# feihoo87/waveforms

Hardware: AMD Instinct MI355X
Metric: Msamples/s (all channels) (higher is better)
Workload: dtype f64; 1 GPU; sampler256: 256 ch/GPU x 1e+07 pts, 100 gaussian+DRAG pulses/ch, seeds 1000+c (SURVEY 8(d) C4/C5 channel spec), grid mode; channels_per_gpu=256, channels_total=256, points_per_channel=10000000, output=device (HBM) buffer, parallelism=channel-block-per-rank x1, no data-path collective

## Files before the change

### include/wfk.h

```cpp
#ifndef WFK_H
#define WFK_H

#include <stddef.h>
#include <stdint.h>

#ifdef __cplusplus
extern "C" {
#endif

#define WFK_ABI_VERSION 2

#define WFK_OK 0
#define WFK_EINVAL (-1)
#define WFK_EUNSUP (-2)
#define WFK_EHIP   (-3)
#define WFK_ENOMEM (-4)
#define WFK_ETIMEOUT (-5)

enum {
  WFK_LINEAR = 1, WFK_GAUSSIAN = 2, WFK_ERF = 3, WFK_COS = 4, WFK_SINC = 5,
  WFK_EXP = 6, WFK_INTERP = 7, WFK_LINEARCHIRP = 8, WFK_EXPONENTIALCHIRP = 9,
  WFK_HYPERBOLICCHIRP = 10, WFK_COSH = 11, WFK_SINH = 12, WFK_DRAG = 13,
  WFK_MOLLIFIER = 14, WFK_D_GAUSSIAN = 15, WFK_DRAG_SIN = 16, WFK_DRAG_SINX = 17,
  WFK_SAMPLED = 1000
// ... 55 lines not shown

int wfk_plan_create_grid(const wfk_program* prog, const wfk_grid* grid,
                         wfk_plan** out);
int wfk_plan_create_tlist(const wfk_program* prog, const double* t_host,
                          int64_t n, wfk_plan** out);
int wfk_grid_detect(const double* t_host, int64_t n, wfk_grid* grid);
int wfk_grid_detect_runs(const double* t_host, int64_t n, int64_t min_len, int32_t max_runs,
                         int64_t* starts, wfk_grid* grids);
int wfk_plan_destroy(wfk_plan* plan);
int wfk_plan_get_info(const wfk_plan* plan, wfk_plan_info* info);
int wfk_plan_member_index(const wfk_plan* plan, int32_t member, int64_t* idx,
                          int32_t cap);
int wfk_plan_channel_is_complex(const wfk_plan* plan, int32_t channel);
const char* wfk_plan_kernel_name(const wfk_plan* plan, int out_kind);
int64_t wfk_plan_table_bytes(const wfk_plan* plan);
int wfk_plan_launch(wfk_plan* plan, void* out_dev, int64_t ch_stride,
                    int out_kind, uint32_t flags, void* hip_stream);
int wfk_plan_run_host(wfk_plan* plan, void* out_host, int64_t ch_stride,
                      int out_kind);

int wfk_fir_plan_create(const double* ker_host, int32_t K, int64_t n,
                        int32_t batch, int kind ,
                        wfk_fir_plan** out);
int wfk_fir_plan_create_rows(const double* kers_host, int32_t K, int64_t n,
                             int32_t batch, int kind ,
                             wfk_fir_plan** out);
int wfk_fir_apply(wfk_fir_plan* plan, const void* in_dev, int64_t in_stride,
                  void* out_dev, int64_t out_stride, void* hip_stream);
int wfk_fir_plan_destroy(wfk_fir_plan* plan);

// ... 119 lines not shown
```

### waveforms_amd/_engine.py

```python
from __future__ import annotations

import ctypes as C
import importlib.util
import os

import numpy as np

from ._flatten import Program, wfk_grid, wfk_program

_HERE = os.path.dirname(os.path.abspath(__file__))
LIB_PATH = os.environ.get('WFK_LIB') or os.path.join(_HERE, 'csrc', 'libwfk_hip.so')

OUT_F64, OUT_F32, OUT_C128, OUT_C64 = 0, 1, 2, 3
ACCUMULATE = 1
_KIND_OF = {np.dtype(np.float64): OUT_F64, np.dtype(np.float32): OUT_F32,
            np.dtype(np.complex128): OUT_C128, np.dtype(np.complex64): OUT_C64}
_DTYPE_OF = {v: k for k, v in _KIND_OF.items()}

E_UNSUP = -2
E_TIMEOUT = -5


class wfk_plan_info(C.Structure):
    _fields_ = [('n_channels', C.c_int32), ('n', C.c_int64), ('tile', C.c_int32),
# ... 22 lines not shown
        l = C.CDLL(LIB_PATH)
        l.wfk_last_error.restype = C.c_char_p
        P, I64, I32, VP = C.POINTER, C.c_int64, C.c_int32, C.c_void_p
        l.wfk_plan_create_grid.argtypes = [P(wfk_program), P(wfk_grid), P(VP)]
        l.wfk_plan_create_tlist.argtypes = [P(wfk_program), VP, I64, P(VP)]
        l.wfk_grid_detect.argtypes = [VP, I64, P(wfk_grid)]
        l.wfk_grid_detect_runs.argtypes = [VP, I64, I64, I32, VP, P(wfk_grid)]
        l.wfk_plan_destroy.argtypes = [VP]
        l.wfk_plan_get_info.argtypes = [VP, P(wfk_plan_info)]
        l.wfk_plan_member_index.argtypes = [VP, I32, VP, I32]
        l.wfk_plan_channel_is_complex.argtypes = [VP, I32]
        l.wfk_plan_kernel_name.argtypes = [VP, C.c_int]
        l.wfk_plan_kernel_name.restype = C.c_char_p
        l.wfk_plan_table_bytes.argtypes = [VP]
        l.wfk_plan_table_bytes.restype = C.c_int64
        l.wfk_plan_launch.argtypes = [VP, VP, I64, C.c_int, C.c_uint32, VP]
        l.wfk_plan_run_host.argtypes = [VP, VP, I64, C.c_int]
        l.wfk_fir_plan_create.argtypes = [VP, I32, I64, I32, C.c_int, P(VP)]
        l.wfk_fir_plan_create_rows.argtypes = [VP, I32, I64, I32, C.c_int, P(VP)]
        l.wfk_chain_plan_create_rows.argtypes = [P(wfk_program), P(wfk_grid), VP, I32, C.c_int, P(VP)]
        l.wfk_fir_apply.argtypes = [VP, VP, I64, VP, I64, VP]
        l.wfk_fir_plan_destroy.argtypes = [VP]
        l.wfk_chain_plan_create.argtypes = [P(wfk_program), P(wfk_grid), VP, I32, C.c_int, P(VP)]
        l.wfk_chain_is_fused.argtypes = [VP]
        l.wfk_chain_unfused_reason.argtypes = [VP]
        l.wfk_chain_unfused_reason.restype = C.c_char_p
        l.wfk_chain_kernel_name.argtypes = [VP]
        l.wfk_chain_kernel_name.restype = C.c_char_p
        l.wfk_chain_table_bytes.argtypes = [VP]
        l.wfk_chain_table_bytes.restype = I64
# ... 146 lines not shown
        self.n = int(info.n)
        self.n_channels = int(info.n_channels)

    def member_index(self, member: int) -> np.ndarray:
        nb = len(self.prog.member_bounds(member))
        idx = np.empty(nb, dtype=np.int64)
        check(lib().wfk_plan_member_index(self._h, member, idx.ctypes.data, nb))
        return idx

    def kernel_name(self, dtype=np.float64) -> str:
        return lib().wfk_plan_kernel_name(self._h, _KIND_OF[np.dtype(dtype)]).decode()

    def table_bytes(self) -> int:
        return int(lib().wfk_plan_table_bytes(self._h))

    def launch(self, out_ptr: int, ch_stride: int, kind: int, accumulate=False,
               stream: int = 0):
        check(lib().wfk_plan_launch(self._h, out_ptr, ch_stride, kind,
                                    ACCUMULATE if accumulate else 0, stream))

    def run_host(self, dtype=np.float64) -> np.ndarray:
        dtype = np.dtype(dtype)
        out = pinned_empty((self.n_channels, self.n), dtype)
        if out.size:
            check(lib().wfk_plan_run_host(self._h, out.ctypes.data, self.n,
                                          _KIND_OF[dtype]))
        return out

    def run_host_into(self, out: np.ndarray):
        if out.size != self.n_channels * self.n or not out.flags.c_contiguous or not out.flags.writeable:
# ... 407 lines not shown
```

### waveforms_amd/csrc/wfk_api.cpp

```cpp
#include <hip/hip_runtime.h>

#include <algorithm>
#include <cstring>
#include <map>
#include <mutex>
#include <thread>
#include <new>
#include <string>
#include <vector>

#include "wfk.h"
#include "wfk_host.h"
#include "wfk_internal.h"

static thread_local std::string g_err;

#define HIP_TRY(expr)                                                                 \
  do {                                                                                \
    hipError_t e_ = (expr);                                                           \
    if (e_ != hipSuccess)                                                             \
      return wfk_fail(WFK_EHIP, std::string(#expr) + ": " + hipGetErrorString(e_));   \
  } while (0)

namespace {
// ... 76 lines not shown
  }
};

struct wfk_plan {
  HostPlan h;
  bool on_device = false;
  void* d_tables = nullptr;
  size_t tables_cap = 0;
  DevChannel* d_channels = nullptr;
  DevPiece* d_pieces = nullptr;
  double* d_params = nullptr;
  double* d_pool = nullptr;
  int32_t* d_chunk_first = nullptr;
  int32_t* d_lean_chunk_first = nullptr;
  int32_t* d_f32_chunk_first = nullptr;
  double* d_tlist = nullptr;
  ShortUnit* d_units = nullptr;
  uint32_t* d_slots = nullptr;
  void* d_scratch = nullptr;
  size_t scratch_bytes = 0;
  size_t scratch_cap = 0;
  int dev = 0;
  bool async_launch = false;
};

static int plan_upload(wfk_plan* p, const double* tlist) {
  if (!wfk_have_device()) {
    p->on_device = false;
    return WFK_OK;
  }
  const HostPlan& h = p->h;
  DevTables t;
  const size_t o_ch = t.add(h.channels);
  const size_t o_pc = t.add(h.pieces.data(), h.shortp && !h.mixed ? 0 : h.pieces.size() * sizeof(DevPiece));
  const size_t o_pa = t.add(h.params), o_po = t.add(h.pool), o_cf = t.add(h.chunk_first);
  const size_t o_lf = t.add(h.lean_chunk_first), o_ff = t.add(h.f32_chunk_first);
  const size_t o_un = t.add(h.s_units), o_sl = t.add(h.s_slots);
  const size_t b_tl = tlist ? (size_t)h.n * sizeof(double) : 0;
  const size_t o_tl = t.reserve(b_tl), total = t.total();
  HIP_TRY(dev_cache().get(total, &p->d_tables, &p->tables_cap, &p->dev));
  char* base = static_cast<char*>(p->d_tables);
  p->d_channels = t.at<DevChannel>(base, o_ch);
  p->d_pieces = t.at<DevPiece>(base, o_pc);
  p->d_params = t.at<double>(base, o_pa);
  p->d_pool = t.at<double>(base, o_po);
  p->d_chunk_first = t.at<int32_t>(base, o_cf);
  p->d_lean_chunk_first = t.at<int32_t>(base, o_lf);
  p->d_f32_chunk_first = t.at<int32_t>(base, o_ff);
  p->d_units = t.at<ShortUnit>(base, o_un);
  p->d_slots = t.at<uint32_t>(base, o_sl);
  p->d_tlist = tlist ? t.at<double>(base, o_tl) : nullptr;
  const std::vector<char>& stage = t.image();
  if (o_tl) HIP_TRY(hipMemcpy(base, stage.data(), o_tl, hipMemcpyHostToDevice));
  if (b_tl) HIP_TRY(hipMemcpy(base + o_tl, tlist, b_tl, hipMemcpyHostToDevice));
  p->on_device = true;
  return WFK_OK;
}

extern "C" {

void wfk_internal_set_error(const char* msg) { g_err = msg ? msg : ""; }

int wfk_abi_version(void) { return WFK_ABI_VERSION; }

const char* wfk_last_error(void) { return g_err.c_str(); }
// ... 32 lines not shown
    if (grid && prog && prog->n_channels >= 32 && prog->n_pieces >= 8192) {
      int nt = (int)std::min<unsigned>(16u, std::max(1u, std::thread::hardware_concurrency()));
      if (const char* e = std::getenv("WFK_COMPILE_THREADS")) nt = std::atoi(e);
      nt = std::min(nt, prog->n_channels / 8);
      if (nt > 1) rc = wfk_compile_blocks(prog, grid, nt, p->h, err);
    }
    if (rc == WFK_RETRY_STD) rc = wfk_compile(prog, grid, tlist, n, p->h, err);
  } catch (...) {
    delete p;
    throw;
  }
  if (rc) {
    delete p;
    return wfk_fail(rc, err);
  }
  std::vector<double> grid_t;
  const char* nopw = std::getenv("WFK_NO_POINTWISE_GRID");
  if (grid && p->h.short_gave_up && grid->n > 0 && grid->n <= ((int64_t)1 << 24) && !(nopw && nopw[0] == '1')) {
    try {
      grid_t.resize((size_t)grid->n);
      wfk_internal_grid_times(grid, grid_t.data());
      HostPlan h2;
      std::string err2;
      TlistNsGuard ns_guard(WFK_NS_TLIST_SMALL);
      const int rc2 = wfk_compile(prog, nullptr, grid_t.data(), grid->n, h2, err2);
      if (rc2 == WFK_OK) {
        h2.grid_as_tlist = true;
        h2.t0 = p->h.t0; h2.step = p->h.step; h2.last = p->h.last;
        h2.has_last = p->h.has_last; h2.i0 = p->h.i0;
        p->h = std::move(h2);
// ... 36 lines not shown
}

int wfk_plan_create_tlist(const wfk_program* prog, const double* t_host, int64_t n,
                          wfk_plan** out) {
  if (!t_host && n > 0) return wfk_fail(WFK_EINVAL, "null t_host");
  static const double dummy = 0.0;
  return plan_create(prog, nullptr, t_host ? t_host : &dummy, n, out);
}

int wfk_plan_destroy(wfk_plan* p) {
  if (!p) return WFK_OK;
  if (p->d_tables || p->d_scratch) {
    DeviceGuard guard(p->dev);
    if (p->async_launch) (void)hipDeviceSynchronize();
    dev_cache().put(p->d_tables, p->tables_cap, p->dev);
    dev_cache().put(p->d_scratch, p->scratch_cap, p->dev);
  }
  delete p;
  return WFK_OK;
}

int wfk_plan_get_info(const wfk_plan* p, wfk_plan_info* info) {
  if (!p || !info) return wfk_fail(WFK_EINVAL, "null argument");
  info->n_channels = p->h.n_channels;
  info->n = p->h.n;
  info->tile = p->h.tile;
  info->n_tiles = p->h.shortp ? (int64_t)p->h.s_units.size() : p->h.chunks_per_ch * p->h.n_channels;
  info->n_pieces = (int32_t)p->h.pieces.size();
  info->param_doubles = (int64_t)p->h.params.size();
  info->n_fast = p->h.n_fast;
// ... 15 lines not shown
  if (!p || channel < 0 || channel >= p->h.n_channels) return wfk_fail(WFK_EINVAL, "bad channel");
  return p->h.channel_complex[channel];
}

void wfk_internal_plan_tables(const wfk_plan* p, const HostPlan** h, const double** d_params) {
  *h = p ? &p->h : nullptr;
  *d_params = p && p->on_device ? p->d_params : nullptr;
}

int64_t wfk_plan_table_bytes(const wfk_plan* p) {
  if (!p) return wfk_fail(WFK_EINVAL, "null plan");
  const HostPlan& h = p->h;
  size_t b = h.channels.size() * sizeof(DevChannel) + h.params.size() * sizeof(double) + h.pool.size() * sizeof(double);
  if (h.shortp) b += h.s_units.size() * sizeof(ShortUnit) + h.s_slots.size() * sizeof(uint32_t);
  if (!h.shortp || h.mixed) b += h.pieces.size() * sizeof(DevPiece) + (h.chunk_first.size() + h.lean_chunk_first.size()) * sizeof(int32_t);
  return (int64_t)b;
}

const char* wfk_plan_kernel_name(const wfk_plan* p, int out_kind) {
  if (!p || out_kind < 0 || out_kind > 3) return "";
  static thread_local std::string name;
  const char* T = (out_kind == WFK_OUT_F32 || out_kind == WFK_OUT_C64) ? "float" : "double";
  const char* cplx = (out_kind == WFK_OUT_C128 || out_kind == WFK_OUT_C64) ? "true" : "false";
  const HostPlan& h = p->h;
  const bool f32 = out_kind == WFK_OUT_F32 || out_kind == WFK_OUT_C64;
  auto general = [&](bool tl, bool g, bool d, int ns) {
    const std::string tail = std::string(cplx) + "," + (tl ? "true" : "false") + "," + (g ? "true" : "false") + "," +
                             (d ? "true" : "false") + "," + std::to_string(ns) + ">";
    return f32 && (tl || g || d) ? "wfk_sample_wide<" + tail : std::string("wfk_sample<") + T + "," + tail;
  };
  if (h.shortp) {
// ... 5 lines not shown
  }
  const std::string lean_name = std::string("wfk_sample_lean<") + T + "," + cplx + "," + std::to_string(h.ns) +
      (h.n_corr > 0 && out_kind != WFK_OUT_F32 && out_kind != WFK_OUT_C64
           ? std::string(",true,") + std::to_string(h.lean_fam >= 1 ? 1 : 0) + ">"
           : std::string(",false,") + std::to_string(h.lean_fam) + ">");
  if (!h.tlist && h.lean) {
    name = lean_name;
  } else {
    const bool tl_full = h.tlist && (h.n_direct > 0 || h.n_generic > 0);
    const bool direct = tl_full || (!h.tlist && h.n_direct > 0), generic = direct || (!h.tlist && h.n_generic > 0);
    name = general(h.tlist, generic, direct, h.ns);
    if (h.mixed && h.tlist) name = general(true, false, false, h.ns) + " + " + name;
    else if (h.mixed) name = lean_name + " + " + name;
  }
  return name.c_str();
}

static int plan_launch_part(wfk_plan* p, void* out_dev, int64_t ch_stride, int out_kind, uint32_t flags,
                            void* hip_stream, int part, int nparts, int64_t* s_lo, int64_t* s_hi) {
  if (!p || (!out_dev && p->h.n > 0)) return wfk_fail(WFK_EINVAL, "null plan or output");
  if (!p->on_device)
    return wfk_fail(WFK_EHIP, "plan has no device tables (no HIP device was visible at plan creation)");
  if (ch_stride < p->h.n) return wfk_fail(WFK_EINVAL, "ch_stride smaller than samples per channel");
  if (s_lo) { *s_lo = 0; *s_hi = p->h.n; }
  if (p->h.n == 0 || p->h.n_channels == 0) return WFK_OK;
  if (nparts > 1 && (p->h.n_channels != 1 || p->h.mixed)) return wfk_fail(WFK_EINVAL, "partial launch of a multi-channel or mixed plan");
  auto sub = [&](int64_t total, int64_t& base, int64_t& count) {
    base = total * part / nparts;
    count = total * (part + 1) / nparts - base;
  };
// ... 72 lines not shown
    a.mixed = 1;
  } else if (p->h.mixed && p->h.tlist) {
    KArgs l = a;
    l.mixed = 1;
    rc = wfk_launch_sampler(l, p->h.n_channels, out_kind, true, p->h.ns, false, false, false, hip_stream, err);
    if (rc) return wfk_fail(rc, err);
    a.mixed = 1;
  } else if (p->h.mixed) {
    KArgs l = a;
    l.mixed = 1;
    l.chunk_first = p->d_lean_chunk_first;
    l.chunks_per_ch = p->h.lean_chunks_per_ch;
    l.n_chunks = p->h.lean_chunks_per_ch * p->h.n_channels;
    l.tiles_per_chunk = p->h.lean_tiles_per_chunk;
    if (f32_lean) use_f32_chunks(l);
    rc = wfk_launch_sampler(l, p->h.n_channels, out_kind, false, p->h.ns, true, false, false, hip_stream, err);
    if (rc) return wfk_fail(rc, err);
    a.mixed = 1;
  }
  if (nparts > 1) {
    const int64_t all = a.n_chunks;
    sub(all, a.chunk_base, a.n_chunks);
    const int64_t tile = (int64_t)(p->h.lean ? 64 : WFK_WG) * p->h.ns, span = tile * a.tiles_per_chunk;
    if (s_lo) {
      *s_lo = std::min<int64_t>(p->h.n, a.chunk_base * span);
      *s_hi = std::min<int64_t>(p->h.n, (a.chunk_base + a.n_chunks) * span);
    }
    if (a.n_chunks == 0) return WFK_OK;
  }
  rc = wfk_launch_sampler(a, p->h.n_channels, out_kind, p->h.tlist, p->h.ns, p->h.lean,
                          p->h.n_generic > 0 || (p->h.tlist && p->h.n_direct > 0),
                          p->h.n_direct > 0 || (p->h.tlist && p->h.n_generic > 0),
                          hip_stream, err);
// ... 252 lines not shown
```

### waveforms_amd/csrc/wfk_compile.cpp

```cpp
#include <algorithm>
#include <chrono>
#include <cmath>
#include <cstdio>
#include <cstdlib>
#include <cstring>
#include <atomic>
#include <map>
#include <string>
#include <thread>
#include <vector>

#include "wfk.h"
#include "wfk_internal.h"

namespace {

struct TimeAxis {
  const wfk_grid* g;
  const double* t;
  int64_t n;
  double at(int64_t i) const {
    if (t) return t[i];
    if (g->has_last && i == g->n - 1) return g->last;
    volatile double m = (double)(i + g->i0) * g->step;
// ... 1996 lines not shown
  H.foreign_frac = frac_sum / (double)P->n_channels;
  H.pool_real = !H.pool.empty();
  if (H.pool.empty()) H.pool.assign(1, 0.0);
  if (H.shortp) {
    const int64_t nu = (int64_t)H.s_units.size();
    H.s_units_per_chunk = (int32_t)std::min<int64_t>(6, std::max<int64_t>(1, nu / 8192));
    if (const char* e = std::getenv("WFK_SH_UPC")) {
      const int v = std::atoi(e);
      if (v >= 1 && v <= 64) H.s_units_per_chunk = v;
    }
    if (H.s_slots.empty()) H.s_slots.push_back(0);
  }
  return WFK_OK;
}

namespace {

struct GridProbe {
  const double* t;
  int64_t n;
  double t0;
  double at(int64_t i, double step) const { return (double)i * step + t0; }
  int64_t first_mismatch(double step, int64_t a, int64_t b, int* sign) const {
    for (int64_t c = a; c < b; c += 1024) {
      const int64_t e = std::min(b, c + 1024);
      int bad = 0;
      const double dc = (double)c;
      const double* tc = t + c;
      const int len = (int)(e - c);
      for (int k = 0; k < len; ++k) bad |= ((dc + (double)k) * step + t0) != tc[k];
// ... 220 lines not shown
```

### waveforms_amd/csrc/wfk_internal.h

```cpp
#pragma once
#include <stdint.h>

#define WFK_WG 256
#define WFK_NS_GRID 16
#define WFK_NS_TLIST 8
#define WFK_NS_TLIST_SMALL 1
#define WFK_TLIST_SMALL_N (1 << 20)
#define WFK_LDS_DOUBLES 2048
#define WFK_FREC 10
#define WFK_BLK_HDR 2
#define WFK_TERM_HDR 4
#define WFK_OP_TERM 1
#define WFK_OP_FCE 2

#define WFK_FCE_REC 22
#define WFK_FCE_W 1
#define WFK_FCE_SREF 2
#define WFK_FCE_SLIN 3
#define WFK_FCE_DEG 4
#define WFK_FCE_PACK(deg, carrier, imag, env, f32ok) ((deg) | ((carrier) << 2) | ((imag) << 3) | ((env) << 4) | ((f32ok) << 6))
#define WFK_FCE_WORD(rec) (reinterpret_cast<const int*>(rec)[2 * WFK_FCE_DEG])
#define WFK_FCE_TABOFF(fl) (((fl) >> 8) & 0x7FF)
#define WFK_FCE_STOFF(fl) ((((fl) >> 19) & 63) * 128)
#define WFK_FCE_HAS_CS (1 << 25)
// ... 31 lines not shown
#endif
#ifndef WFK_LEAN_PAR
#define WFK_LEAN_PAR 896
#endif
#define WFK_CHAIN_PAR 2048
#ifndef WFK_LEAN_RESEED
#define WFK_LEAN_RESEED 8
#endif
#define WFK_LEAN_RESEED_F32 32
#ifndef WFK_LEAN_RESEED_CS
#define WFK_LEAN_RESEED_CS 64
#endif
#define WFK_LEAN_TPC 5
#define WFK_LEAN_TPC_F32 20

#define WFK_PF_HAS_TERMS 1
#define WFK_PF_LEAN 2

#define WFK_SH_R 16
#define WFK_SH_LCAP 1008
#define WFK_SH_SUB 4096
#define WFK_SH_FILL 1008
#define WFK_SH_ERFTAB 512
#define WFK_SH_OP1 12
#define WFK_SH_OP3 16
#define WFK_SH_LAST 64
#define WFK_PF_SHORT 4
#define WFK_SH_SLOT(drec16, o, len) \
  ((uint32_t)(drec16) | ((uint32_t)(o) << 16) | ((uint32_t)((len) - 1) << 26) | 0x80000000u)
#define WFK_SH_DREC_MAX 0xffff
// ... 57 lines not shown
  int64_t n;
  int64_t chunks_per_ch;
  int64_t n_chunks;
  int64_t chunk_base;
  int32_t tiles_per_chunk;
  int32_t accumulate;
  double t0, step, last;
  int32_t has_last, pad;
  int32_t lean_par, lean_ops;
  int32_t corr;
  int32_t reseed;
  int32_t lean_fam;
  int32_t wavepriv;
  int32_t mixed;
  int64_t i0;
};

#ifdef __cplusplus
#include <string>
#include <vector>
struct wfk_program;
struct wfk_grid;
struct wfk_plan;
struct wfk_fir_plan;

struct HostPlan {
  bool tlist = false;
  int32_t n_channels = 0;
  int64_t n = 0;
  double t0 = 0, step = 0, last = 0;
// ... 6 lines not shown
  std::vector<double> params, pool;
  std::vector<int32_t> chunk_first;
  std::vector<std::vector<int64_t>> member_idx;
  std::vector<uint8_t> channel_complex;
  int32_t n_fast = 0, n_direct = 0, n_fused = 0, n_generic = 0;
  int32_t n_corr = 0;
  bool lean = false;
  int32_t lean_fam = 0;
  bool mixed = false;
  int32_t lean_tile = 0, lean_tiles_per_chunk = 1;
  int64_t lean_chunks_per_ch = 0;
  std::vector<int32_t> lean_chunk_first;
  int32_t f32_tiles_per_chunk = 0;
  int64_t f32_chunks_per_ch = 0;
  std::vector<int32_t> f32_chunk_first;
  int32_t lean_par = 0, lean_ops = 0;
  bool shortp = false;
  int32_t max_block_len = 0;
  double foreign_frac = 0.0;
  double mean_piece_len = 0.0;
  bool short_gave_up = false;
  bool grid_as_tlist = false;
  bool short_has_fmul = false;
  int32_t short_fam = 0;
  bool short_corr = false;
  bool short_needs_corr = false;
  bool pool_real = false;
  std::vector<ShortUnit> s_units;
  std::vector<uint32_t> s_slots;
  int32_t s_lds_samples = 0, s_units_per_chunk = 1;
};

int wfk_compile(const wfk_program* prog, const wfk_grid* grid, const double* tlist,
                int64_t n, HostPlan& out, std::string& err);

int wfk_compile_geom(const wfk_program* prog, const wfk_grid* grid, int lane_stride, int ns,
                     HostPlan& out, std::string& err);
#define WFK_RETRY_STD 1
int wfk_compile_blocks(const wfk_program* prog, const wfk_grid* grid, int nthreads, HostPlan& out, std::string& err);

struct ShortWin {
  int64_t rec0;
  int64_t e0;
  int32_t cnt, pad;
  int32_t ccnt, pad2;
};
#define WFK_PLAN_FOREIGN_ONLY 0x80000000u
#define WFK_CW_ENTRY(drec, o, len) ((uint32_t)(drec) | ((uint32_t)(o) << 16) | ((uint32_t)((len) - 1) << 28))
int wfk_chain_windows(const HostPlan& H, int64_t n, int64_t hop, int64_t lead, int64_t half, int64_t npairs,
                      std::vector<ShortWin>& wins, std::vector<uint32_t>& entries, std::string& err);

void wfk_internal_keep_mixed_short(bool on);
void wfk_internal_tlist_ns(int ns);
void wfk_internal_grid_times(const wfk_grid* g, double* out);
void wfk_internal_no_short_fmul(bool on);

int wfk_launch_sampler(const KArgs& a, int32_t n_channels, int out_kind, bool tlist, int ns,
                       bool lean, bool generic, bool direct, void* stream, std::string& err);
int wfk_launch_short(const SArgs& a, int out_kind, void* stream, std::string& err);

extern "C" {
void wfk_internal_set_error(const char* msg);
void wfk_internal_plan_tables(const wfk_plan* p, const HostPlan** h, const double** d_params);
int wfk_internal_plan_launch_foreign(wfk_plan* p, void* out_dev, int64_t ch_stride, int out_kind, void* hip_stream);
void wfk_internal_fir_tables(const wfk_fir_plan* p, const void** kspec, const void** tw, int* fused, int* nseg,
                             int* K, int* lead);
int64_t wfk_internal_fir_krow(const wfk_fir_plan* p);
int wfk_internal_fir_fused_launch(int kind, const void* in, int64_t in_stride, void* out, int64_t out_stride,
                                  const void* hspec, const void* tw, int64_t n, int M, int K, int lead, int64_t nblk,
                                  int32_t batch, int accumulate, void* stream, int64_t hspec_row_stride);
int wfk_internal_fir_fused_len(void);
}
#endif
// ... 1 lines not shown
```

### waveforms_amd/csrc/wfk_kernels.hip

```cpp
#include <hip/hip_runtime.h>

#include <string>
#include <type_traits>
#include <utility>

#include "wfk.h"
#include "wfk_internal.h"

namespace {

__device__ __forceinline__ int uni(int v) { return __builtin_amdgcn_readfirstlane(v); }
__device__ __forceinline__ int64_t uni64(int64_t v) {
  const uint32_t lo = __builtin_amdgcn_readfirstlane((uint32_t)v);
  const uint32_t hi = __builtin_amdgcn_readfirstlane((uint32_t)((uint64_t)v >> 32));
  return (int64_t)(((uint64_t)hi << 32) | lo);
}
#define WFK_CONST __attribute__((address_space(4)))
template <typename V>
__device__ __forceinline__ V cload(const void* base, int byte_off) {
  return *reinterpret_cast<const WFK_CONST V*>(reinterpret_cast<uintptr_t>(base) + byte_off);
}
__device__ __forceinline__ DevPiece load_piece(const DevPiece* p) {
  DevPiece P;
  P.start = cload<int64_t>(p, offsetof(DevPiece, start));
// ... 1179 lines not shown
  const bool full = P.start <= w0 && P.stop >= w0 + 64 * NS;
  const bool clip = C.do_clip && (P.flags & WFK_PF_HAS_TERMS);
  if (full && !clip && !a.accumulate)
    store_tile_impl<T, CPLX, NS, true, NT, E>(a, C, P, tr, tc, w0, lane, acc, acci);
  else
    store_tile_impl<T, CPLX, NS, false, NT, E>(a, C, P, tr, tc, w0, lane, acc, acci);
}

__device__ __forceinline__ int64_t xcd_chunk(const KArgs& a) {
  const int64_t b = blockIdx.x;
  const int64_t per = (a.n_chunks + 7) >> 3;
  const int64_t c = (b & 7) * per + (b >> 3);
  return c < a.n_chunks ? a.chunk_base + c : -1;
}

template <typename T, bool CPLX, int NS, bool CORR, int FAM>
#ifndef WFK_LEAN_WAVES
#define WFK_LEAN_WAVES 3
#endif
#ifndef WFK_LEAN_WAVES_F32
#define WFK_LEAN_WAVES_F32 4
#endif
__global__ void __launch_bounds__(64, (sizeof(T) == 4 ? WFK_LEAN_WAVES_F32 : WFK_LEAN_WAVES) - (CPLX ? 1 : 0) -
                                          (CORR && sizeof(T) == 8 && !CPLX ? 1 : 0))
wfk_sample_lean(const KArgs a) {
  extern __shared__ __attribute__((aligned(16))) double s_dyn[];
  double* const s_par = s_dyn;
  double* const s_st = s_dyn + a.lean_par;
  constexpr int WT = 64 * NS;
  using OutR = typename OutOps<T>::Real;
  using OutC = typename OutOps<T>::Cplx;

  const int lane = threadIdx.x;
  const int64_t chunk = xcd_chunk(a);
  if (chunk < 0) return;
  const int ch = uni((int)(chunk / a.chunks_per_ch));
  const int64_t cc = uni64(chunk - (int64_t)ch * a.chunks_per_ch);
  const DevChannel C = a.channels[ch];
  int p = uni(a.chunk_first[chunk]);
  DevPiece cur = load_piece(a.pieces + p);
  int64_t staged = -1;
  int state_piece = -1;
  int64_t state_w0 = -1;
  int since_seed = 0;
  int cs_age = 0;

  OutR* const outr = uniptr(reinterpret_cast<OutR*>(a.out) + (int64_t)ch * a.ch_stride);
  OutC* const outc = uniptr(reinterpret_cast<OutC*>(a.out) + (int64_t)ch * a.ch_stride);

  for (int tt = 0; tt < a.tiles_per_chunk; ++tt) {
    const int64_t w0 = uni64((cc * a.tiles_per_chunk + tt) * WT);
    if (w0 >= a.n) break;
    const int64_t w1 = w0 + WT < a.n ? w0 + WT : a.n;
    const int64_t j0 = w0 + lane;
    while (p < C.piece_end - 1 && cur.stop <= w0) {
      p = uni(p + 1);
      cur = load_piece(a.pieces + p);
    }

    for (int q = p;;) {
      const DevPiece P = cur;
      if (P.start >= w1) break;
      T acc[NS], acci[CPLX ? NS : 1];
      WFK_EACH(NS, k) acc[k] = (T)0; WFK_END
      WFK_EACH(CPLX ? NS : 1, k) acci[k] = (T)0; WFK_END
      const bool mine = !a.mixed || P.n_blk == 0 || (P.flags & WFK_PF_LEAN);
      if (P.n_blk != 0 && mine) {
        if (P.par_off != staged) {
          __syncthreads();
          for (int i = lane; i < P.first_len; i += 64) s_par[i] = a.params[P.par_off + i];
          __syncthreads();
          staged = P.par_off;
        }
        const int nops = uni((int)s_par[1]);
        double x = grid_time(a, j0);
        if (C.tshift != 0.0) x = x - C.tshift;
        const bool valid = state_piece == q && state_w0 == w0;
        const bool carried = valid && since_seed < a.reseed;
        if (!carried) {
          bool seed_cs = true;
          if constexpr (!CORR) {
            seed_cs = !valid || cs_age >= WFK_LEAN_RESEED_CS;
          }
          if (seed_cs) cs_age = 0;
          for (int op = 0; op < nops; ++op) {
            const double* srec = s_par + WFK_BLK_HDR + op * WFK_FCE_REC;
            const int sfl = uni(WFK_FCE_WORD(srec));
            if constexpr (!CORR) {
              if (!seed_cs && (sfl & (WFK_FCE_HAS_CS | WFK_FCE_HAS_GR | WFK_FCE_CHIRP)) == WFK_FCE_HAS_CS) continue;
            }
            if constexpr (FAM >= 2) {
              if (sfl & WFK_FCE_CHIRP) {
                const ChirpSeeds cd = chirp_make_seeds(srec, x, sfl);
                double* ct = s_st + WFK_FCE_STOFF(sfl) + lane;
                ct[0] = cd.c; ct[64] = cd.s; ct[128] = cd.wc; ct[192] = cd.ws;
                if (sfl & WFK_FCE_HAS_GR) { ct[256] = cd.g; ct[320] = cd.r; }
                continue;
              }
            }
            if constexpr (FAM >= 3) {
              if ((sfl & 0x32) == 0x32) continue;
            }
            const FceSeeds sd = fce_make_seeds<CORR>(srec, x, sfl);
// ... 311 lines not shown
    if (TLIST && !generic && !direct) { hipLaunchKernelGGL((wfk_sample_wide<CPLX, TLIST, false, false, NS>), g, b, 0, s, a); return hipGetLastError() == hipSuccess ? 0 : -1; }
    if (TLIST || direct) { hipLaunchKernelGGL((wfk_sample_wide<CPLX, TLIST, true, true, NS>), g, b, 0, s, a); return hipGetLastError() == hipSuccess ? 0 : -1; }
    if (generic) { hipLaunchKernelGGL((wfk_sample_wide<CPLX, false, true, false, NS>), g, b, 0, s, a); return hipGetLastError() == hipSuccess ? 0 : -1; }
  }
  if (TLIST && !generic && !direct)
    hipLaunchKernelGGL((wfk_sample<T, CPLX, TLIST, false, false, NS>), g, b, 0, s, a);
  else if (TLIST || direct)
    hipLaunchKernelGGL((wfk_sample<T, CPLX, TLIST, true, true, NS>), g, b, 0, s, a);
  else if (generic)
    hipLaunchKernelGGL((wfk_sample<T, CPLX, false, true, false, NS>), g, b, 0, s, a);
  else
    hipLaunchKernelGGL((wfk_sample<T, CPLX, false, false, false, NS>), g, b, 0, s, a);
  return hipGetLastError() == hipSuccess ? 0 : -1;
}

}

int wfk_launch_sampler(const KArgs& a, int32_t n_channels, int out_kind, bool tlist, int ns, bool lean,
                       bool generic, bool direct, void* stream, std::string& err) {
  if (a.chunk_base < 0 || a.chunk_base + a.n_chunks > (int64_t)n_channels * a.chunks_per_ch) { err = "chunk range outside the plan"; return WFK_EINVAL; }
  const int64_t blocks = ((a.n_chunks + 7) >> 3) << 3;
  if (blocks == 0) return WFK_OK;
  if (blocks > 0x7fffffffLL) { err = "grid too large"; return WFK_EINVAL; }
  hipStream_t s = (hipStream_t)stream;
  int rc;
  if (!tlist) {
    switch (out_kind) {
      case WFK_OUT_F64: rc = launch<double, false, false, WFK_NS_GRID>(a, blocks, s, lean, generic, direct); break;
      case WFK_OUT_F32: rc = launch<float, false, false, WFK_NS_GRID>(a, blocks, s, lean, generic, direct); break;
      case WFK_OUT_C128: rc = launch<double, true, false, WFK_NS_GRID>(a, blocks, s, lean, generic, direct); break;
// ... 24 lines not shown
```

Before: 805,900 Msamples/s.

## Precompute per-chunk oscillator and envelope seeds in a cached device table

Adds a pre-pass kernel that, on first launch, computes libm-based cos/sin/gaussian seeds at each lean chunk's first sample and stores them in a persistent device table. The main kernel's first reseed per chunk then reads the table and derives per-lane values with angle-doubling rotations and truncated Taylor exponentials instead of calling transcendental functions. Ops are admitted only when the Taylor argument bounds hold. This adds table memory, a one-time pre-pass, and event synchronisation across streams, and it reuses the table on later launches of the same plan.

```diff
diff --git a/include/wfk.h b/include/wfk.h
--- a/include/wfk.h
+++ b/include/wfk.h
@@ -93,6 +93,9 @@
 int wfk_plan_channel_is_complex(const wfk_plan* plan, int32_t channel);
 const char* wfk_plan_kernel_name(const wfk_plan* plan, int out_kind);
 int64_t wfk_plan_table_bytes(const wfk_plan* plan);
+int64_t wfk_plan_seed_map(const wfk_plan* plan, int map, int32_t* chunk_piece, int32_t* slot_first, int64_t cap,
+                          int64_t* chunk_samples);
+int wfk_plan_seed_ops(const wfk_plan* plan, int32_t piece, int32_t* admitted, int32_t cap, int64_t* range);
 int wfk_plan_launch(wfk_plan* plan, void* out_dev, int64_t ch_stride,
                     int out_kind, uint32_t flags, void* hip_stream);
 int wfk_plan_run_host(wfk_plan* plan, void* out_host, int64_t ch_stride,
diff --git a/waveforms_amd/_engine.py b/waveforms_amd/_engine.py
--- a/waveforms_amd/_engine.py
+++ b/waveforms_amd/_engine.py
@@ -60,6 +60,9 @@
         l.wfk_plan_kernel_name.restype = C.c_char_p
         l.wfk_plan_table_bytes.argtypes = [VP]
         l.wfk_plan_table_bytes.restype = C.c_int64
+        l.wfk_plan_seed_map.argtypes = [VP, C.c_int, VP, VP, I64, P(I64)]
+        l.wfk_plan_seed_map.restype = I64
+        l.wfk_plan_seed_ops.argtypes = [VP, I32, VP, I32, VP]
         l.wfk_plan_launch.argtypes = [VP, VP, I64, C.c_int, C.c_uint32, VP]
         l.wfk_plan_run_host.argtypes = [VP, VP, I64, C.c_int]
         l.wfk_fir_plan_create.argtypes = [VP, I32, I64, I32, C.c_int, P(VP)]
@@ -236,6 +239,23 @@
     def table_bytes(self) -> int:
         return int(lib().wfk_plan_table_bytes(self._h))
 
+    def seed_map(self, which: int = 0):
+        samples = C.c_int64(0)
+        n = int(check(lib().wfk_plan_seed_map(self._h, which, None, None, 0, C.byref(samples))))
+        if n == 0:
+            return None
+        piece, first = np.empty(n, np.int32), np.empty(n + 1, np.int32)
+        lib().wfk_plan_seed_map(self._h, which, piece.ctypes.data, first.ctypes.data, n + 1, None)
+        return piece, first, int(samples.value)
+
+    def seed_ops(self, piece: int):
+        rng = np.zeros(2, np.int64)
+        adm = np.zeros(64, np.int32)
+        n = lib().wfk_plan_seed_ops(self._h, piece, adm.ctypes.data, 64, rng.ctypes.data)
+        if n < 0:
+            raise IndexError(piece)
+        return adm[:n].copy(), (int(rng[0]), int(rng[1]))
+
     def launch(self, out_ptr: int, ch_stride: int, kind: int, accumulate=False,
                stream: int = 0):
         check(lib().wfk_plan_launch(self._h, out_ptr, ch_stride, kind,
diff --git a/waveforms_amd/csrc/wfk_api.cpp b/waveforms_amd/csrc/wfk_api.cpp
--- a/waveforms_amd/csrc/wfk_api.cpp
+++ b/waveforms_amd/csrc/wfk_api.cpp
@@ -114,6 +114,16 @@
   int32_t* d_chunk_first = nullptr;
   int32_t* d_lean_chunk_first = nullptr;
   int32_t* d_f32_chunk_first = nullptr;
+  int32_t* d_seed_first[3] = {nullptr, nullptr, nullptr};
+  double* d_seed_lane = nullptr;
+  struct SeedTab {
+    void* tab = nullptr;
+    size_t cap = 0;
+    hipEvent_t ready = nullptr;
+    void* stream = nullptr;
+    bool built = false;
+  } seed[3];
+  std::mutex seed_mu;
   double* d_tlist = nullptr;
   ShortUnit* d_units = nullptr;
   uint32_t* d_slots = nullptr;
@@ -136,6 +146,8 @@
   const size_t o_pa = t.add(h.params), o_po = t.add(h.pool), o_cf = t.add(h.chunk_first);
   const size_t o_lf = t.add(h.lean_chunk_first), o_ff = t.add(h.f32_chunk_first);
   const size_t o_un = t.add(h.s_units), o_sl = t.add(h.s_slots);
+  const size_t o_s0 = t.add(h.seed_first[0]), o_s1 = t.add(h.seed_first[1]), o_s2 = t.add(h.seed_first[2]);
+  const size_t o_sn = t.add(h.seed_lane);
   const size_t b_tl = tlist ? (size_t)h.n * sizeof(double) : 0;
   const size_t o_tl = t.reserve(b_tl), total = t.total();
   HIP_TRY(dev_cache().get(total, &p->d_tables, &p->tables_cap, &p->dev));
@@ -149,6 +161,10 @@
   p->d_f32_chunk_first = t.at<int32_t>(base, o_ff);
   p->d_units = t.at<ShortUnit>(base, o_un);
   p->d_slots = t.at<uint32_t>(base, o_sl);
+  p->d_seed_first[0] = h.seed_first[0].empty() ? nullptr : t.at<int32_t>(base, o_s0);
+  p->d_seed_first[1] = h.seed_first[1].empty() ? nullptr : t.at<int32_t>(base, o_s1);
+  p->d_seed_first[2] = h.seed_first[2].empty() ? nullptr : t.at<int32_t>(base, o_s2);
+  p->d_seed_lane = t.at<double>(base, o_sn);
   p->d_tlist = tlist ? t.at<double>(base, o_tl) : nullptr;
   const std::vector<char>& stage = t.image();
   if (o_tl) HIP_TRY(hipMemcpy(base, stage.data(), o_tl, hipMemcpyHostToDevice));
@@ -211,6 +227,7 @@
     delete p;
     return wfk_fail(rc, err);
   }
+  wfk_seed_tables(p->h);
   std::vector<double> grid_t;
   const char* nopw = std::getenv("WFK_NO_POINTWISE_GRID");
   if (grid && p->h.short_gave_up && grid->n > 0 && grid->n <= ((int64_t)1 << 24) && !(nopw && nopw[0] == '1')) {
@@ -277,6 +294,10 @@
     DeviceGuard guard(p->dev);
     if (p->async_launch) (void)hipDeviceSynchronize();
     dev_cache().put(p->d_tables, p->tables_cap, p->dev);
+    for (auto& st : p->seed) {
+      if (st.tab) dev_cache().put(st.tab, st.cap, p->dev);
+      if (st.ready) (void)hipEventDestroy(st.ready);
+    }
     dev_cache().put(p->d_scratch, p->scratch_cap, p->dev);
   }
   delete p;
@@ -322,7 +343,39 @@
   size_t b = h.channels.size() * sizeof(DevChannel) + h.params.size() * sizeof(double) + h.pool.size() * sizeof(double);
   if (h.shortp) b += h.s_units.size() * sizeof(ShortUnit) + h.s_slots.size() * sizeof(uint32_t);
   if (!h.shortp || h.mixed) b += h.pieces.size() * sizeof(DevPiece) + (h.chunk_first.size() + h.lean_chunk_first.size()) * sizeof(int32_t);
+  b += h.seed_lane.size() * sizeof(double);
+  for (const auto& f : h.seed_first)
+    if (!f.empty()) b += f.size() * sizeof(int32_t) + (size_t)f.back() * WFK_SEED_SLOT * sizeof(double);
   return (int64_t)b;
+}
+
+int64_t wfk_plan_seed_map(const wfk_plan* p, int map, int32_t* chunk_piece, int32_t* slot_first, int64_t cap,
+                          int64_t* chunk_samples) {
+  if (!p || map < 0 || map > 2) return wfk_fail(WFK_EINVAL, "bad plan or map");
+  const HostPlan& h = p->h;
+  const std::vector<int32_t>& first = h.seed_first[map];
+  if (first.empty()) return 0;
+  const std::vector<int32_t>& cf = map == 0 ? h.chunk_first : map == 1 ? h.lean_chunk_first : h.f32_chunk_first;
+  const int64_t tpc = map == 0 ? h.tiles_per_chunk : map == 1 ? h.lean_tiles_per_chunk : h.f32_tiles_per_chunk;
+  if (chunk_samples) *chunk_samples = tpc * 64 * h.ns;
+  for (int64_t i = 0; i < cap && i < (int64_t)cf.size(); ++i)
+    if (chunk_piece) chunk_piece[i] = cf[(size_t)i];
+  for (int64_t i = 0; i < cap && i < (int64_t)first.size(); ++i)
+    if (slot_first) slot_first[i] = first[(size_t)i];
+  return (int64_t)cf.size();
+}
+
+int wfk_plan_seed_ops(const wfk_plan* p, int32_t piece, int32_t* admitted, int32_t cap, int64_t* range) {
+  if (!p || piece < 0 || piece >= (int32_t)p->h.pieces.size()) return -1;
+  const HostPlan& h = p->h;
+  const DevPiece& D = h.pieces[(size_t)piece];
+  if (range) { range[0] = D.start; range[1] = D.stop; }
+  if (h.tlist || h.shortp || D.n_blk == 0 || !(h.lean || (h.mixed && (D.flags & WFK_PF_LEAN)))) return 0;
+  const double* blk = h.params.data() + D.par_off;
+  const int nops = (int)blk[1];
+  for (int op = 0; op < nops && op < cap; ++op)
+    if (admitted) admitted[op] = WFK_FCE_HIWORD(blk + WFK_BLK_HDR + op * WFK_FCE_REC) < 0 ? 1 : 0;
+  return nops;
 }
 
 const char* wfk_plan_kernel_name(const wfk_plan* p, int out_kind) {
@@ -358,6 +411,37 @@
     else if (h.mixed) name = lean_name + " + " + name;
   }
   return name.c_str();
+}
+
+static int seed_attach(wfk_plan* p, int m, KArgs& k, void* hip_stream, std::string& err) {
+  const std::vector<int32_t>& first = p->h.seed_first[m];
+  if (first.empty() || first.back() == 0 || p->h.n_seed_ops == 0) return WFK_OK;
+  wfk_plan::SeedTab& st = p->seed[m];
+  std::lock_guard<std::mutex> lock(p->seed_mu);
+  k.seed_first = p->d_seed_first[m];
+  k.seed_lane = p->d_seed_lane;
+  if (!st.built) {
+    const size_t bytes = (size_t)first.back() * WFK_SEED_SLOT * sizeof(double);
+    DeviceGuard guard(p->dev);
+    int dev = 0;
+    if (!st.tab && dev_cache().get(bytes, &st.tab, &st.cap, &dev) != hipSuccess) {
+      err = "out of device memory for the seed table";
+      return WFK_EHIP;
+    }
+    if (!st.ready && hipEventCreateWithFlags(&st.ready, hipEventDisableTiming) != hipSuccess) {
+      err = "hipEventCreate failed";
+      return WFK_EHIP;
+    }
+    const int rc = wfk_launch_seed_prepass(k, p->h.n_channels, p->h.ns, static_cast<double*>(st.tab), hip_stream, err);
+    if (rc) return rc;
+    if (hipEventRecord(st.ready, (hipStream_t)hip_stream) != hipSuccess) { err = "hipEventRecord failed"; return WFK_EHIP; }
+    st.stream = hip_stream;
+    st.built = true;
+  } else if (st.stream != hip_stream) {
+    if (hipStreamWaitEvent((hipStream_t)hip_stream, st.ready, 0) != hipSuccess) { err = "hipStreamWaitEvent failed"; return WFK_EHIP; }
+  }
+  k.seed_tab = static_cast<const double*>(st.tab);
+  return WFK_OK;
 }
 
 static int plan_launch_part(wfk_plan* p, void* out_dev, int64_t ch_stride, int out_kind, uint32_t flags,
@@ -460,9 +544,15 @@
     l.n_chunks = p->h.lean_chunks_per_ch * p->h.n_channels;
     l.tiles_per_chunk = p->h.lean_tiles_per_chunk;
     if (f32_lean) use_f32_chunks(l);
+    rc = seed_attach(p, f32_lean ? 2 : 1, l, hip_stream, err);
+    if (rc) return wfk_fail(rc, err);
     rc = wfk_launch_sampler(l, p->h.n_channels, out_kind, false, p->h.ns, true, false, false, hip_stream, err);
     if (rc) return wfk_fail(rc, err);
     a.mixed = 1;
+  }
+  if (p->h.lean) {
+    rc = seed_attach(p, f32_lean ? 2 : 0, a, hip_stream, err);
+    if (rc) return wfk_fail(rc, err);
   }
   if (nparts > 1) {
     const int64_t all = a.n_chunks;
diff --git a/waveforms_amd/csrc/wfk_compile.cpp b/waveforms_amd/csrc/wfk_compile.cpp
--- a/waveforms_amd/csrc/wfk_compile.cpp
+++ b/waveforms_amd/csrc/wfk_compile.cpp
@@ -8,6 +8,7 @@
 #include <map>
 #include <string>
 #include <thread>
+#include <unordered_set>
 #include <vector>
 
 #include "wfk.h"
@@ -2034,6 +2035,81 @@
   return WFK_OK;
 }
 
+void wfk_seed_tables(HostPlan& H) {
+  for (auto& v : H.seed_first) v.clear();
+  H.seed_lane.clear();
+  H.n_seed_ops = 0;
+  if (H.tlist || H.shortp || !(H.lean || H.mixed) || H.n_corr > 0 || H.n == 0) return;
+  if (const char* e = std::getenv("WFK_LEAN_LIBM_SEEDS")) if (e[0] == '1') return;
+  const double dt = H.step;
+  auto time_at = [&](int64_t j) { return (double)(j + H.i0) * H.step + H.t0; };
+  std::unordered_set<int64_t> seen;
+  for (int32_t c = 0; c < H.n_channels; ++c) {
+    const DevChannel& C = H.channels[(size_t)c];
+    for (int32_t pi = C.piece_begin; pi < C.piece_end; ++pi) {
+      const DevPiece& D = H.pieces[(size_t)pi];
+      if (D.n_blk == 0 || !(H.lean || (D.flags & WFK_PF_LEAN))) continue;
+      double* blk = H.params.data() + D.par_off;
+      const int nops = (int)blk[1];
+      const bool again = !seen.insert(D.par_off).second;
+      const double xa = time_at(D.start) - C.tshift, xb = time_at(D.stop) - C.tshift;
+      for (int op = 0; op < nops; ++op) {
+        double* rec = blk + WFK_BLK_HDR + op * WFK_FCE_REC;
+        uint32_t w[2];
+        std::memcpy(w, &rec[WFK_FCE_DEG], sizeof w);
+        const uint32_t fl = w[0];
+        const int env = (fl >> 4) & 3;
+        bool ok = rec[0] == (double)WFK_OP_FCE && env <= 1 && !(fl & 128) &&
+                  !(fl & (WFK_FCE_CHIRP | WFK_FCE_BANK | WFK_FCE_OWNMUL)) && (fl & (WFK_FCE_HAS_CS | WFK_FCE_HAS_GR));
+        double e2 = 0.0, e3 = 0.0, k1 = 0.0, k0 = 0.0;
+        if (ok && env == 1) {
+          if (fl & WFK_FCE_EXPENV) {
+            k0 = rec[WFK_FCE_SIGMA] * dt;
+            ok = 63.0 * std::fabs(k0) <= WFK_SEED_MAX_G;
+          } else {
+            const double sigma = rec[WFK_FCE_SIGMA], b = dt / sigma;
+            const double vmax = std::max(std::fabs((xa - rec[WFK_FCE_SG]) / sigma), std::fabs((xb - rec[WFK_FCE_SG]) / sigma));
+            e2 = -b * b; k1 = -2.0 * b / sigma; e3 = -2.0 * rec[WFK_FCE_H] * b;
+            ok = 63.0 * (2.0 * vmax * std::fabs(b) + 63.0 * b * b) <= WFK_SEED_MAX_G && 63.0 * std::fabs(e3) <= WFK_SEED_MAX_R;
+          }
+        }
+        if (again) {
+          if (!ok && (w[1] & WFK_SEED_ADMIT)) { w[1] = 0; std::memcpy(&rec[WFK_FCE_DEG], w, sizeof w); --H.n_seed_ops; }
+          continue;
+        }
+        w[1] = 0;
+        if (ok) {
+          w[1] = WFK_SEED_ADMIT | (uint32_t)(H.seed_lane.size() / WFK_SEED_LANE);
+          double L[WFK_SEED_LANE];
+          for (int k = 0; k < 6; ++k) {
+            const double th = rec[WFK_FCE_W] * dt * (double)(1 << k);
+            L[2 * k] = std::cos(th); L[2 * k + 1] = std::sin(th);
+          }
+          L[12] = e2; L[13] = e3; L[14] = k1; L[15] = k0;
+          H.seed_lane.insert(H.seed_lane.end(), L, L + WFK_SEED_LANE);
+          ++H.n_seed_ops;
+        }
+        std::memcpy(&rec[WFK_FCE_DEG], w, sizeof w);
+      }
+    }
+  }
+  if (H.n_seed_ops == 0) { H.seed_lane.clear(); return; }
+  auto slots = [&](const std::vector<int32_t>& chunk_first, std::vector<int32_t>& first) {
+    first.assign(chunk_first.size() + 1, 0);
+    int64_t at = 0;
+    for (size_t k = 0; k < chunk_first.size(); ++k) {
+      first[k] = (int32_t)at;
+      const DevPiece& D = H.pieces[(size_t)chunk_first[k]];
+      if (D.n_blk != 0 && (H.lean || (D.flags & WFK_PF_LEAN))) at += (int64_t)H.params[(size_t)D.par_off + 1];
+      if (at > 0x7fffffff) { first.clear(); return; }
+    }
+    first[chunk_first.size()] = (int32_t)at;
+  };
+  if (H.lean) slots(H.chunk_first, H.seed_first[0]);
+  if (H.mixed && !H.lean_chunk_first.empty()) slots(H.lean_chunk_first, H.seed_first[1]);
+  if (!H.f32_chunk_first.empty()) slots(H.f32_chunk_first, H.seed_first[2]);
+}
+
 namespace {
 
 struct GridProbe {
diff --git a/waveforms_amd/csrc/wfk_internal.h b/waveforms_amd/csrc/wfk_internal.h
--- a/waveforms_amd/csrc/wfk_internal.h
+++ b/waveforms_amd/csrc/wfk_internal.h
@@ -69,6 +69,15 @@
 #define WFK_LEAN_TPC 5
 #define WFK_LEAN_TPC_F32 20
 
+#define WFK_SEED_SLOT 4
+#define WFK_SEED_LANE 16
+#define WFK_SEED_ADMIT 0x80000000u
+#define WFK_SEED_DEG_G 14
+#define WFK_SEED_DEG_R 8
+#define WFK_SEED_MAX_G 0.5
+#define WFK_SEED_MAX_R 0.06
+#define WFK_FCE_HIWORD(rec) (reinterpret_cast<const int*>(rec)[2 * WFK_FCE_DEG + 1])
+
 #define WFK_PF_HAS_TERMS 1
 #define WFK_PF_LEAN 2
 
@@ -156,6 +165,9 @@
   int32_t wavepriv;
   int32_t mixed;
   int64_t i0;
+  const double* seed_tab;
+  const int32_t* seed_first;
+  const double* seed_lane;
 };
 
 #ifdef __cplusplus
@@ -192,6 +204,9 @@
   int32_t f32_tiles_per_chunk = 0;
   int64_t f32_chunks_per_ch = 0;
   std::vector<int32_t> f32_chunk_first;
+  std::vector<int32_t> seed_first[3];
+  std::vector<double> seed_lane;
+  int32_t n_seed_ops = 0;
   int32_t lean_par = 0, lean_ops = 0;
   bool shortp = false;
   int32_t max_block_len = 0;
@@ -216,6 +231,7 @@
                      HostPlan& out, std::string& err);
 #define WFK_RETRY_STD 1
 int wfk_compile_blocks(const wfk_program* prog, const wfk_grid* grid, int nthreads, HostPlan& out, std::string& err);
+void wfk_seed_tables(HostPlan& H);
 
 struct ShortWin {
   int64_t rec0;
@@ -235,6 +251,7 @@
 
 int wfk_launch_sampler(const KArgs& a, int32_t n_channels, int out_kind, bool tlist, int ns,
                        bool lean, bool generic, bool direct, void* stream, std::string& err);
+int wfk_launch_seed_prepass(const KArgs& a, int32_t n_channels, int ns, double* tab, void* stream, std::string& err);
 int wfk_launch_short(const SArgs& a, int out_kind, void* stream, std::string& err);
 
 extern "C" {
diff --git a/waveforms_amd/csrc/wfk_kernels.hip b/waveforms_amd/csrc/wfk_kernels.hip
--- a/waveforms_amd/csrc/wfk_kernels.hip
+++ b/waveforms_amd/csrc/wfk_kernels.hip
@@ -1217,6 +1217,47 @@
   return c < a.n_chunks ? a.chunk_base + c : -1;
 }
 
+template <int N>
+__device__ __forceinline__ double seed_exp(double x) {
+  constexpr double inv_fact[17] = {1.0, 1.0, 1.0 / 2, 1.0 / 6, 1.0 / 24, 1.0 / 120, 1.0 / 720, 1.0 / 5040, 1.0 / 40320,
+                                   1.0 / 362880, 1.0 / 3628800, 1.0 / 39916800, 1.0 / 479001600, 1.0 / 6227020800.0,
+                                   1.0 / 87178291200.0, 1.0 / 1307674368000.0, 1.0 / 20922789888000.0};
+  double p = inv_fact[N];
+  WFK_EACH(N, i) p = __builtin_fma(p, x, inv_fact[N - 1 - i]); WFK_END
+  return p;
+}
+__device__ __attribute__((noinline)) void seed_from_table(const double* sb_, const double* lr_, const double* srec_, int sfl,
+                                                          double x0, int lane, double* st_) {
+  const double* const sb = reinterpret_cast<const double*>(uni64(reinterpret_cast<int64_t>(sb_)));
+  const double* const lr = reinterpret_cast<const double*>(uni64(reinterpret_cast<int64_t>(lr_)));
+  sfl = uni(sfl);
+  using LdsD = __attribute__((address_space(3))) double;
+  LdsD* st = (LdsD*)st_;
+  const LdsD* const srec = (const LdsD*)srec_;
+  if (sfl & WFK_FCE_HAS_CS) {
+    double c = cload<double>(sb, 0), s = cload<double>(sb, 8);
+    WFK_EACH(6, k)
+      const double pc = cload<double>(lr, 16 * k), ps = cload<double>(lr, 16 * k + 8);
+      if (lane & (1 << k)) {
+        const double t = c * ps;
+        c = c * pc;
+        c = __builtin_fma(-s, ps, c);
+        s = __builtin_fma(s, pc, t);
+      }
+    WFK_END
+    st[0] = c;
+    st[64] = s;
+    st += 128;
+  }
+  if (sfl & WFK_FCE_HAS_GR) {
+    const double l = (double)lane;
+    const double e2 = cload<double>(lr, 96), e3 = cload<double>(lr, 104), k1 = cload<double>(lr, 112), k0 = cload<double>(lr, 120);
+    const double e1 = __builtin_fma(k1, x0 - srec[WFK_FCE_SG], k0);
+    st[0] = cload<double>(sb, 16) * seed_exp<WFK_SEED_DEG_G>(__builtin_fma(e2, l, e1) * l);
+    st[64] = cload<double>(sb, 24) * seed_exp<WFK_SEED_DEG_R>(e3 * l);
+  }
+}
+
 template <typename T, bool CPLX, int NS, bool CORR, int FAM>
 #ifndef WFK_LEAN_WAVES
 #define WFK_LEAN_WAVES 3
@@ -1247,6 +1288,7 @@
   int64_t state_w0 = -1;
   int since_seed = 0;
   int cs_age = 0;
+  int slot0 = a.seed_tab != nullptr ? cload<int32_t>(a.seed_first + chunk, 0) : -1;
 
   OutR* const outr = uniptr(reinterpret_cast<OutR*>(a.out) + (int64_t)ch * a.ch_stride);
   OutC* const outc = uniptr(reinterpret_cast<OutC*>(a.out) + (int64_t)ch * a.ch_stride);
@@ -1264,6 +1306,8 @@
     for (int q = p;;) {
       const DevPiece P = cur;
       if (P.start >= w1) break;
+      const int slot = slot0;
+      slot0 = -1;
       T acc[NS], acci[CPLX ? NS : 1];
       WFK_EACH(NS, k) acc[k] = (T)0; WFK_END
       WFK_EACH(CPLX ? NS : 1, k) acci[k] = (T)0; WFK_END
@@ -1290,6 +1334,16 @@
             const double* srec = s_par + WFK_BLK_HDR + op * WFK_FCE_REC;
             const int sfl = uni(WFK_FCE_WORD(srec));
             if constexpr (!CORR) {
+              if (slot >= 0) {
+                const int hw = uni(WFK_FCE_HIWORD(srec));
+                if (hw < 0) {
+                  const double x0 = __builtin_bit_cast(double, uni64(__builtin_bit_cast(int64_t, x)));
+                  seed_from_table(a.seed_tab + (int64_t)WFK_SEED_SLOT * (slot + op),
+                                  a.seed_lane + (int64_t)WFK_SEED_LANE * (hw & 0x7fffffff), srec, sfl, x0, lane,
+                                  s_st + WFK_FCE_STOFF(sfl) + lane);
+                  continue;
+                }
+              }
               if (!seed_cs && (sfl & (WFK_FCE_HAS_CS | WFK_FCE_HAS_GR | WFK_FCE_CHIRP)) == WFK_FCE_HAS_CS) continue;
             }
             if constexpr (FAM >= 2) {
@@ -1631,6 +1685,41 @@
   return hipGetLastError() == hipSuccess ? 0 : -1;
 }
 
+__global__ void __launch_bounds__(256) wfk_seed_prepass(const KArgs a, double* tab, int wt) {
+  const int64_t chunk = (int64_t)blockIdx.x * 256 + threadIdx.x;
+  if (chunk >= a.n_chunks) return;
+  const int ch = (int)(chunk / a.chunks_per_ch);
+  const int64_t w0 = (chunk - (int64_t)ch * a.chunks_per_ch) * a.tiles_per_chunk * wt;
+  if (w0 >= a.n) return;
+  const DevChannel C = a.channels[ch];
+  const DevPiece P = a.pieces[a.chunk_first[chunk]];
+  if (P.n_blk == 0 || (a.mixed && !(P.flags & WFK_PF_LEAN))) return;
+  const double* blk = a.params + P.par_off;
+  const int nops = (int)blk[1];
+  double x = grid_time(a, w0);
+  if (C.tshift != 0.0) x = x - C.tshift;
+  double* out = tab + (int64_t)WFK_SEED_SLOT * a.seed_first[chunk];
+  for (int op = 0; op < nops; ++op, out += WFK_SEED_SLOT) {
+    const double* rec = blk + WFK_BLK_HDR + op * WFK_FCE_REC;
+    if (WFK_FCE_HIWORD(rec) >= 0) continue;
+    const FceSeeds sd = fce_make_seeds<false>(rec, x, WFK_FCE_WORD(rec));
+    out[0] = sd.c; out[1] = sd.s; out[2] = sd.g; out[3] = sd.r;
+  }
+}
+
+}
+
+int wfk_launch_seed_prepass(const KArgs& a, int32_t n_channels, int ns, double* tab, void* stream, std::string& err) {
+  if (!a.seed_first || !tab || a.chunk_base != 0 || a.n_chunks != (int64_t)n_channels * a.chunks_per_ch) {
+    err = "seed pre-pass: not a whole chunk map";
+    return WFK_EINVAL;
+  }
+  const int64_t blocks = (a.n_chunks + 255) / 256;
+  if (blocks == 0) return WFK_OK;
+  if (blocks > 0x7fffffffLL) { err = "grid too large"; return WFK_EINVAL; }
+  hipLaunchKernelGGL(wfk_seed_prepass, dim3((unsigned)blocks), dim3(256), 0, (hipStream_t)stream, a, tab, 64 * ns);
+  if (hipGetLastError() != hipSuccess) { err = "seed pre-pass launch failed"; return WFK_EHIP; }
+  return WFK_OK;
 }
 
 int wfk_launch_sampler(const KArgs& a, int32_t n_channels, int out_kind, bool tlist, int ns, bool lean,
```

After: 768,100 Msamples/s. -4.7%, worse.
